# jseppanen/azalea

Measured on AMD Instinct MI355X. Metric: mcts_sims_per_sec, higher is better.
Workload: dtype f16x3 (fp32 operands split hi+lo f16, fp32 accumulate)

## Files before the change

azalea_amd/_lib.py:

```python
import ctypes as C
import logging
import os
import subprocess

_HERE = os.path.dirname(os.path.abspath(__file__))
LIB_PATH = os.path.join(_HERE, "libazx_hip.so")

MAX_BOARD = 13
CELL_STRIDE = 192
MAX_BATCH = 16
ROW_METRICS = 8


def record_bytes(cells):
    return (16 + 5 * cells + 15) // 16 * 16

EVAL_RESNET, EVAL_UNIFORM, EVAL_UNIFORM_HASH, EVAL_EXTERNAL = 0, 1, 2, 3
FLAG_NO_COMPACT = 1
FLAG_RANDOM_REFLECT = 2
FLAG_TOWER_F16 = 4
EEXTERNAL = -7


class AzxError(RuntimeError):
# ... 63 lines not shown
    "azx_get_status": (C.c_int, [_vp, _i32p]),
    "azx_get_tree_nodes": (C.c_int, [_vp, _i32p]),
    "azx_get_games": (C.c_int, [_vp, _i32p, _i32p, _i32p, _i32p]),
    "azx_advance": (C.c_int, [_vp, _i32p]),
    "azx_tree_dump": (C.c_int, [_vp, C.c_int, C.c_int, _i32p, _i32p, _i32p, _f32p, _f32p, _f32p, _i32p, _i32p]),
    "azx_forward": (C.c_int, [_vp, C.c_int, C.c_int, _i32p, _i32p, _f32p, _f32p]),
    "azx_hex_replay": (C.c_int, [C.c_int, C.c_int, C.c_int, _i32p, _i32p, C.c_int, _i32p, _i32p, _u64p, _i32p]),
    "azx_play": (C.c_int, [_vp, C.c_int64, C.c_int64, C.c_int64, _i32p, _i32p, _i32p, _f32p, _f32p, _i64p, C.POINTER(PlayStats)]),
    "azx_play_row_metrics": (C.c_int, [_vp, C.c_int64, _f32p, _i64p]),
    "azx_play_steps": (C.c_int, [_vp, C.c_int64, C.POINTER(PlayStats)]),
    "azx_replay_create": (C.c_int, [_vp, C.c_int64]),
    "azx_replay_state": (C.c_int, [_vp, _i64p, _i64p, _i64p]),
    "azx_replay_set_state": (C.c_int, [_vp, C.c_int64, C.c_int64]),
    "azx_replay_put": (C.c_int, [_vp, C.c_int64, _i32p, _i32p, _i32p, _f32p, _f32p]),
    "azx_replay_fill": (C.c_int, [_vp, C.c_int64, C.c_int64, _i64p, C.POINTER(PlayStats)]),
    "azx_play_device": (C.c_int, [_vp, C.c_int64, C.c_int64, _i64p, C.POINTER(PlayStats)]),
    "azx_rows_pack": (C.c_int, [_vp, C.c_int64, C.c_int64, _vp]),
    "azx_replay_put_records": (C.c_int, [_vp, C.c_int64, _vp]),
    "azx_replay_put_records_async": (C.c_int, [_vp, C.c_int64, _vp, _vp]),
    "azx_reserve_cus": (C.c_int, [_vp, C.c_int, C.POINTER(C.c_int)]),
    "azx_replay_collate": (C.c_int, [_vp, C.c_int64, _i64p, _vp, _vp, _vp, _vp, _vp, _vp, _i32p]),
    "azx_replay_collate_async": (C.c_int, [_vp, C.c_int64, _i64p, _vp, _vp, _vp, _vp, _vp, _vp, _vp]),
    "azx_replay_set_mover_view": (C.c_int, [_vp, C.c_int]),
    "azx_replay_set_reflect": (C.c_int, [_vp, C.c_int, C.c_uint64]),
    "azx_selftest_arith": (C.c_int, [C.c_int, C.c_int, _f32p, _f32p, _f32p, _f32p, _f32p]),
    "azx_selftest_divide": (C.c_int, [C.c_int, C.c_int, _f32p, _f32p, _f32p, _f32p]),
    "azx_selftest_dirichlet": (C.c_int, [C.c_int, C.c_double, C.c_int, C.c_int, C.c_uint32, _f32p]),
    "azx_debug_choose": (C.c_int, [_vp, _i32p, _f32p]),
    "azx_debug_counters": (C.c_int, [_vp, _u64p]),
    "azx_debug_counters_raw": (C.c_int, [_vp, _u64p, C.c_int64]),
    "azx_kernel_info": (C.c_int, [_vp, C.c_char_p, C.c_int]),
    "azx_debug_set_queue_cap": (C.c_int, [_vp, C.c_int64]),
    "azx_debug_stagger": (C.c_int, [_vp, _i32p]),
    "azx_stream": (_vp, [_vp]),
    "azx_set_external_evaluator": (C.c_int, [_vp, _vp, _vp]),
    "azx_match_create": (C.c_int, [_vp, _vp, C.POINTER(_vp)]),
    "azx_match_destroy": (None, [_vp]),
    "azx_match_play": (C.c_int, [_vp, C.c_int64, C.c_int64, C.POINTER(C.c_int8), C.POINTER(C.c_int16),
                                 C.POINTER(C.c_int16), C.POINTER(MatchStats)]),
    "azx_tournament_create": (C.c_int, [C.POINTER(_vp), C.c_int, C.POINTER(_vp)]),
    "azx_tournament_destroy": (None, [_vp]),
    "azx_tournament_play": (C.c_int, [_vp, C.c_int, _i32p, _i32p, C.c_int64, C.c_int64, C.c_int32,
                                      C.POINTER(C.c_int8), C.POINTER(C.c_int16), C.POINTER(C.c_int16),
                                      C.POINTER(MatchStats)]),
    "azx_match_set_harvest": (C.c_int, [_vp, C.c_int]),
    "azx_match_set_first_mover": (C.c_int, [_vp, C.c_int]),
    "azx_match_rows": (C.c_int, [_vp, _i64p]),
    "azx_tournament_set_harvest": (C.c_int, [_vp, C.c_int]),
    "azx_tournament_set_first_mover": (C.c_int, [_vp, C.c_int]),
    "azx_tournament_rows": (C.c_int, [_vp, _i64p]),
    "azx_rows_read": (C.c_int, [_vp, C.c_int64, C.c_int64, _i32p, _i32p, _i32p, _f32p, _f32p, _i64p]),
    "azx_openings_check": (C.c_int, [C.c_int, C.c_int, C.c_int, C.POINTER(C.c_int16), _i32p, _i32p, _i32p]),
    "azx_match_set_openings": (C.c_int, [_vp, C.c_int, C.c_int, C.POINTER(C.c_int16), _i32p]),
    "azx_tournament_set_openings": (C.c_int, [_vp, C.c_int, C.c_int, C.POINTER(C.c_int16), _i32p]),
    "azx_set_playout_cap": (C.c_int, [_vp, C.c_double, C.c_int]),
    "azx_playout_cap_is_full": (C.c_int, [C.c_uint64, C.c_int64, C.c_int, C.c_double]),
    "azx_playout_cap_stats": (C.c_int, [_vp, _i64p]),
    "azx_set_resign": (C.c_int, [_vp, C.c_double, C.c_int, C.c_double]),
    "azx_clear_resign": (C.c_int, [_vp]),
    "azx_resign_is_exempt": (C.c_int, [C.c_uint64, C.c_int64, C.c_double]),
    "azx_resign_stats": (C.c_int, [_vp, _i64p]),
    "azx_resign_value": (C.c_int, [_vp, C.POINTER(C.c_float)]),
    "azx_set_early_stop": (C.c_int, [_vp, C.c_int]),
    "azx_early_stop_stats": (C.c_int, [_vp, _i64p]),
    "azx_set_train_targets": (C.c_int, [_vp, C.c_int, C.c_float]),
    "azx_get_train_targets": (C.c_int, [_vp, C.POINTER(C.c_int), C.POINTER(C.c_float)]),
# ... 62 lines not shown
```

azalea_amd/csrc/azx_capi.cpp:

```cpp
#include <hip/hip_runtime.h>

#include <algorithm>
#include <cmath>
#include <cstdarg>
#include <cstdio>
#include <cstdlib>
#include <cstring>
#include <map>
#include <mutex>
#include <string>
#include <vector>

#include "../../include/azx.h"
#include "azx_dev.h"
#include "mcts_kernels.h"
#include "net.h"
#include "train.h"
#include "replay_kernels.h"
#include "ext_kernels.h"
#include "match_kernels.h"
#include "playout_cap.h"
#include "resign.h"

#ifndef AZX_SRC_SHA
#define AZX_SRC_SHA "unknown"
#endif

static thread_local std::string g_err;

static int fail(int code, const char *fmt, ...) {
    char buf[1024];
    va_list ap;
    va_start(ap, fmt);
    vsnprintf(buf, sizeof buf, fmt, ap);
    va_end(ap);
    g_err = buf;
    return code;
}

#define HIPCHECK(expr)                                                                    \
    do {                                                                                  \
        hipError_t _e = (expr);                                                           \
        if (_e != hipSuccess)                                                             \
            return fail(AZX_EHIP, "%s failed: %s (%s:%d)", #expr, hipGetErrorString(_e),  \
                        __FILE__, __LINE__);                                              \
    } while (0)

struct azx_engine {
    azx_config cfg;
    DevEngine d;
    hipStream_t stream = nullptr;
    int reserved_cus = 0;
    std::mutex alloc_mu;
    int num_batches = 0;
    int selects_per_search = 0;
// ... 400 lines not shown
    } else {
        snprintf(tree, sizeof tree, "k_mcts<%d,generic> (BEGIN / APPLY|SELECT / APPLY phases)", S);
        snprintf(play, sizeof play, "%s", !use_pipeline(e) ? "phases + k_choose + k_advance per move, one stream"
                                          : e->stagger     ? "phases + k_choose + k_advance per move, two half-pools on two streams half an evaluation apart (any tower)"
                                                           : "phases + k_choose + k_advance per move, two half-pools on two streams");
    }
    std::string text = std::string("tree=") + tree + "; play=" + play + "; net=" +
                       (e->net ? azx_net_kernel_info(e->net) : "none") +
                       "; switches: AZX_MCTS_GENERIC=" + (e->force_generic ? "1" : "0") +
                       " AZX_NO_PERSISTENT=" + (e->no_persistent ? "1" : "0") +
                       " AZX_PIPELINE=" + (e->pipeline ? "1" : "0") +
                       " AZX_PIPELINE_STAGGER=" + (e->stagger ? "1" : "0") +
                       " reserved_cus=" + std::to_string(e->reserved_cus) +
                       " reflect=" + ((d.flags & AZX_FLAG_RANDOM_REFLECT) ? "on" : "off") +
                       " cap=" + cap_text(e) +
                       " resign=" + resign_text(e) +
                       " estop=" + (e->estop_on ? "on" : "off") +
                       " targets=" + targets_text(e) +
                       "; src=" AZX_SRC_SHA;
    snprintf(buf, (size_t)cap, "%s", text.c_str());
    return (int)text.size();
}

extern "C" int azx_debug_stagger(azx_engine *e, int32_t *out4) {
    if (!e || !out4) return fail(AZX_EINVAL, "null argument");
    ENGINE_GUARD(e);
    memset(out4, 0, 4 * sizeof(int32_t));
    if (!e->stagger_ctr) return AZX_OK;
    HIPCHECK(hipMemcpyAsync(out4, e->stagger_ctr, 4 * sizeof(int32_t), hipMemcpyDeviceToHost, e->stream));
    HIPCHECK(hipStreamSynchronize(e->stream));
    return AZX_OK;
}

extern "C" int azx_debug_set_queue_cap(azx_engine *e, int64_t rows) {
    if (!e || rows < 0) return fail(AZX_EINVAL, "bad argument");
    e->dbg_qcap = rows;
    return AZX_OK;
}

static int check_net_range(azx_engine *e) {
    if (!e->net) return AZX_OK;
    int rc = azx_net_check_range(e->net, e->stream);
    if (rc) g_err = azx_net_error();
    return rc;
}

extern "C" int azx_debug_weights(azx_engine *e, int which, void *out, int64_t cap, int64_t *nbytes, char *name, int name_cap) {
    if (!e) return fail(AZX_EINVAL, "null engine");
    ENGINE_GUARD(e);
    if (!e->net) return fail(AZX_ESTATE, "engine was not created with AZX_EVAL_RESNET");
    int rc = azx_net_debug_weights(e->net, which, out, cap, nbytes, name, name_cap);
    if (rc) g_err = azx_net_error();
    return rc;
}

extern "C" int azx_set_weights(azx_engine *e, int n_tensors, const char *const *names,
                               const void *const *ptrs, const int64_t *counts, int on_device) {
    if (!e) return fail(AZX_EINVAL, "null engine");
    ENGINE_GUARD(e);
    if (!e->net) return fail(AZX_ESTATE, "engine was not created with AZX_EVAL_RESNET");
    int rc = azx_net_set_weights(e->net, n_tensors, names, ptrs, counts, on_device);
    if (rc) g_err = azx_net_error();
    return rc;
}

extern "C" int azx_set_prior_table(azx_engine *e, const float *prior_by_k, int count) {
// ... 2266 lines not shown
```

azalea_amd/csrc/net_kernels.hip:

```cpp
#include "net_priv.h"

#ifndef AZX_NET_ABLATE
#define AZX_NET_ABLATE 0
#endif
#ifndef AZX_SAT_TRACK
#define AZX_SAT_TRACK 1
#endif

#include <cmath>
#include <cstdio>
#include <cstdlib>
#include <cstring>
#include <map>
#include <string>
#include <type_traits>
#include <utility>
#include <vector>

typedef float f32x16 __attribute__((ext_vector_type(16)));

static thread_local std::string g_net_err;
const char *azx_net_error() { return g_net_err.c_str(); }

int azx_net_fail(int code, const char *msg) {
    g_net_err = msg;
    return code;
}
static int nfail(int code, const char *msg) { return azx_net_fail(code, msg); }


template <int C, int MT, int BPB, int MS, int NS>
__global__ __launch_bounds__(256) void k_tower_mfma(NetDev P, const uint8_t *__restrict__ ev_board,
                                                     const int32_t *__restrict__ n_eval_ptr,
// ... 165 lines not shown
#endif

#ifndef F16X3_BPB
#define F16X3_BPB 2
#endif
#ifndef AZX_S16_FENCE
#define AZX_S16_FENCE 1
#endif
typedef float f32x4 __attribute__((ext_vector_type(4)));

__global__ __launch_bounds__(F16X3_BPB * 128, 2) void k_tower_f16x3_s16(NetDev P, const uint8_t *__restrict__ ev_board,
                                                                        const int32_t *__restrict__ n_eval_ptr,
                                                                        int n_eval_host, float *__restrict__ act_out,
                                                                        float *__restrict__ hfeat) {
    constexpr int C = 64, ROWB = 272, MT = 4, NT = 4;
    extern __shared__ __align__(16) unsigned char smem[];
    const int n_eval = n_eval_ptr ? *n_eval_ptr : n_eval_host;
    const int e0 = blockIdx.x * F16X3_BPB;
    if (e0 >= n_eval) return;
    const int tid = threadIdx.x, lane = tid & 63, wave = __builtin_amdgcn_readfirstlane(tid >> 6);
    NT_DECL
    const int wb = wave >> 1, wh = wave & 1;
    const int N = P.N, ncells = P.ncells;
    const int e = e0 + wb;
    const bool live = e < n_eval;
    const int board_b = 128 * ROWB;
    const int zero_off = 0;
    const int x_off = 2 * ROWB + wb * board_b;
    unsigned char *X = smem + x_off;
    const int li = lane & 15, lh = lane >> 4;
    const int lrow = li < 8 ? li ^ 4 : li;
    const int lchunk = 128 * (lh & 1) + 16 * (lh >> 1);

    unsigned long long tapok = 0ull;
    int rbase[MT], ry_[MT], rx_[MT];
#pragma unroll
    for (int m = 0; m < MT; ++m) {
        const int r = 64 * wh + 16 * m + lrow;
        const int ry = r / N, rx = r - ry * N;
        ry_[m] = ry;
        rx_[m] = rx;
        rbase[m] = x_off + r * ROWB + lchunk;
#pragma unroll
        for (int tap = 0; tap < 9; ++tap) {
            const int yy = ry + tap / 3 - 1, xx = rx + tap % 3 - 1;
            if (r < ncells && yy >= 0 && yy < N && xx >= 0 && xx < N) tapok |= 1ull << (tap * 4 + m);
        }
    }
    uint32_t tapok_lo = (uint32_t)tapok, tapok_hi = (uint32_t)(tapok >> 32);
    auto act_offset = [&](int tap, int m) -> int {
        const int delta = ((tap / 3 - 1) * N + (tap % 3 - 1)) * ROWB;
        const uint32_t word = tap < 8 ? tapok_lo : tapok_hi;
        const int mask = (int)(word << (31 - ((tap * 4 + m) & 31))) >> 31;
        return (mask | 0xF0) & (rbase[m] + delta);
    };

    f32x4 res[MT][NT];
    auto load_bias = [&](const float *bias, float4 (&b4)[NT]) {
#pragma unroll
        for (int n = 0; n < NT; ++n) b4[n] = *reinterpret_cast<const float4 *>(bias + 16 * n + 4 * lh);
    };
    float satmax = 0.f;
    auto epilogue = [&](f32x4 (&acc)[MT][NT], const float4 (&bias4)[NT], auto kind_tag) {
        constexpr int kind = decltype(kind_tag)::value;
#pragma unroll
        for (int n = 0; n < NT; ++n) {
            const float4 b4 = bias4[n];
            const float bv[4] = {b4.x, b4.y, b4.z, b4.w};
#pragma unroll
            for (int m = 0; m < MT; ++m) {
                float v4[4];
#pragma unroll
                for (int j = 0; j < 4; ++j) {
                    float v = acc[m][n][j] + bv[j];
                    if (kind == 1) v += res[m][n][j];
                    v = fmaxf(v, 0.0f);
                    if (kind != 0) res[m][n][j] = v;
                    v4[j] = v;
                }
                if (AZX_SAT_TRACK) satmax = fmaxf(fmaxf(satmax, v4[0]), fmaxf(v4[1], fmaxf(v4[2], v4[3])));
                uint2 h4, l4;
                split2_f16(v4[0], v4[1], h4.x, l4.x);
                split2_f16(v4[2], v4[3], h4.y, l4.y);
                unsigned char *pw = X + (64 * wh + 16 * m + lrow) * ROWB + 128 * (lh >> 1) + 16 * n + 8 * (lh & 1);
                *reinterpret_cast<uint2 *>(pw) = h4;
                *reinterpret_cast<uint2 *>(pw + 64) = l4;
            }
        }
    };

    {
        const int NH = N + 2;
        unsigned char *cells = X + 121 * ROWB;
        const uint8_t *bd = ev_board + (size_t)(live ? e : n_eval - 1) * AZX_CELL_STRIDE;
        if (wh == 0) {
            for (int i = lane; i < NH * NH; i += 64) {
                const int y = i / NH - 1, x = i - (y + 1) * NH - 1;
                cells[i] = (y >= 0 && y < N && x >= 0 && x < N) ? bd[y * N + x] : (uint8_t)3;
            }
        }
        for (int i = tid; i < 2 * ROWB / 4; i += F16X3_BPB * 128) reinterpret_cast<uint32_t *>(smem + zero_off)[i] = 0u;
        __syncthreads();
        f32x4 acc[MT][NT];
#pragma unroll
        for (int m = 0; m < MT; ++m)
#pragma unroll
            for (int n = 0; n < NT; ++n) acc[m][n] = f32x4{0.f, 0.f, 0.f, 0.f};
        const uint4 *ws = reinterpret_cast<const uint4 *>(P.Ws16);
        f16x8 wfh[NT], wfl[NT];
#pragma unroll
        for (int n = 0; n < NT; ++n) {
            const uint4 qh = ws[(n * 2) * 64 + lane], ql = ws[(n * 2 + 1) * 64 + lane];
            wfh[n] = *reinterpret_cast<const f16x8 *>(&qh);
            wfl[n] = *reinterpret_cast<const f16x8 *>(&ql);
        }
#pragma unroll
        for (int m = 0; m < MT; ++m) {
            uint32_t onehot = 0u;
            if (64 * wh + 16 * m + lrow < ncells) {
                const unsigned char *c0 = cells + ry_[m] * NH + rx_[m];
#pragma unroll
                for (int tap = 0; tap < 9; ++tap) {
                    const uint32_t v = c0[(tap / 3) * NH + tap % 3];
                    onehot |= (v < 3u ? 1u : 0u) << (3 * tap + v);
                }
            }
            const uint32_t byte = (onehot >> (8 * lh)) & 0xffu;
            uint4 q;
            q.x = ((byte >> 0) & 1u) * 0x3C00u | ((byte >> 1) & 1u) * 0x3C000000u;
            q.y = ((byte >> 2) & 1u) * 0x3C00u | ((byte >> 3) & 1u) * 0x3C000000u;
            q.z = ((byte >> 4) & 1u) * 0x3C00u | ((byte >> 5) & 1u) * 0x3C000000u;
            q.w = ((byte >> 6) & 1u) * 0x3C00u | ((byte >> 7) & 1u) * 0x3C000000u;
            const f16x8 xf = *reinterpret_cast<const f16x8 *>(&q);
#pragma unroll
            for (int n = 0; n < NT; ++n) {
                acc[m][n] = __builtin_amdgcn_mfma_f32_16x16x32_f16(wfh[n], xf, acc[m][n], 0, 0, 0);
                acc[m][n] = __builtin_amdgcn_mfma_f32_16x16x32_f16(wfl[n], xf, acc[m][n], 0, 0, 0);
            }
        }
        float4 sb4[NT];
        load_bias(P.stem_b, sb4);
        __syncthreads();
        epilogue(acc, sb4, std::integral_constant<int, 2>{});
    }
    __syncthreads();
    NT_MARK(0)

    const uint4 *wsrc = reinterpret_cast<const uint4 *>(P.Wh16);
    int stage = 0;
    const int last_stage = P.layers * 18 - 1;
    f16x8 wh_[NT], wl_[NT];
    auto load_w = [&](int st, int nn, int part) {
        const uint4 qq = wsrc[(size_t)min(st, last_stage) * 512 + (nn * 2 + part) * 64 + lane];
        if (part) wl_[nn] = *reinterpret_cast<const f16x8 *>(&qq);
        else wh_[nn] = *reinterpret_cast<const f16x8 *>(&qq);
    };
#pragma unroll
    for (int i = 0; i < 4; ++i) load_w(0, i >> 1, i & 1);
    auto conv_layer = [&](int layer, auto residual_tag) {
        constexpr bool residual = decltype(residual_tag)::value;
        asm volatile("" : "+v"(tapok_lo), "+v"(tapok_hi), "+v"(rbase[0]), "+v"(rbase[1]), "+v"(rbase[2]), "+v"(rbase[3]));
        f32x4 acc[MT][NT];
#pragma unroll
        for (int m = 0; m < MT; ++m)
#pragma unroll
            for (int n = 0; n < NT; ++n) acc[m][n] = f32x4{0.f, 0.f, 0.f, 0.f};
        f16x8 xh[MT], xl[MT];
        auto load_x = [&](int tt, int mm, int part) {
            const unsigned char *pa = smem + act_offset(tt >> 1, mm) + (tt & 1) * 32 + part * 64;
            if (part) xl[mm] = *reinterpret_cast<const f16x8 *>(pa);
            else xh[mm] = *reinterpret_cast<const f16x8 *>(pa);
        };
#pragma unroll
        for (int m = 0; m < MT - 1; ++m) { load_x(0, m, 0); load_x(0, m, 1); }
#pragma unroll
        for (int t = 0; t < 18; ++t) {
#pragma unroll
            for (int h = 0; h < 2; ++h) {
#pragma unroll
                for (int q = 0; q < 24; ++q) {
                    const int m = q / 6, n = 2 * h + (q % 6) / 3, p = q % 3;
                    if (q == 1 || q == 4 || q == 7 || q == 10) {
                        const int idx = (q - 1) / 3;
                        if (h == 0) load_w(stage + t, 2 + (idx >> 1), idx & 1);
                        else load_w(stage + t + 1, idx >> 1, idx & 1);
                    } else if (h == 0 && (q == 13 || q == 16)) {
                        load_x(t, MT - 1, q == 16);
                    } else if (h == 1 && q >= 8 && (q % 6 == 2 || q % 6 == 5)) {
                        if (t + 1 < 18) load_x(t + 1, q / 6 - 1, q % 6 == 5);
                    }
                    const f16x8 wv = p == 1 ? wl_[n] : wh_[n];
                    const f16x8 xv = p == 2 ? xl[m] : xh[m];
                    acc[m][n] = __builtin_amdgcn_mfma_f32_16x16x32_f16(wv, xv, acc[m][n], 0, 0, 0);
#if AZX_S16_FENCE == 2
                    __builtin_amdgcn_sched_barrier(0);
#elif AZX_S16_FENCE == 1
                    if (q % 3 == 2) __builtin_amdgcn_sched_barrier(0);
#elif AZX_S16_FENCE == 3
                    if (q % 6 == 5) __builtin_amdgcn_sched_barrier(0);
#elif AZX_S16_FENCE == 4
                    if (q % 2 == 1) __builtin_amdgcn_sched_barrier(0);
#endif
                }
            }
        }
        stage += 18;
        float4 lb4[NT];
        load_bias(P.bias + layer * C, lb4);
        NT_MARK(2)
        __syncthreads();
        NT_MARK(3)
        epilogue(acc, lb4, std::integral_constant<int, residual ? 1 : 0>{});
        NT_MARK(4)
        __syncthreads();
        NT_MARK(5)
    };
    for (int blk = 0; blk < P.blocks; ++blk) {
        conv_layer(2 * blk, std::false_type{});
        conv_layer(2 * blk + 1, std::true_type{});
    }

    if (hfeat != nullptr) {
        const uint4 *whd = reinterpret_cast<const uint4 *>(P.Whd16);
        f16x8 ah[2], al[2];
#pragma unroll
        for (int ks = 0; ks < 2; ++ks) {
            const uint4 qh = whd[(ks * 2) * 64 + lane], ql = whd[(ks * 2 + 1) * 64 + lane];
            ah[ks] = *reinterpret_cast<const f16x8 *>(&qh);
            al[ks] = *reinterpret_cast<const f16x8 *>(&ql);
        }
        const float4 hb = *reinterpret_cast<const float4 *>(P.hbias16 + 4 * lh);
        const float hbv[4] = {hb.x, hb.y, hb.z, hb.w};
#pragma unroll
        for (int m = 0; m < MT; ++m) {
            f32x4 hacc = f32x4{0.f, 0.f, 0.f, 0.f};
#pragma unroll
            for (int ks = 0; ks < 2; ++ks) {
                const unsigned char *pa = smem + rbase[m] + ks * 32;
                const f16x8 xh = *reinterpret_cast<const f16x8 *>(pa), xl = *reinterpret_cast<const f16x8 *>(pa + 64);
                hacc = __builtin_amdgcn_mfma_f32_16x16x32_f16(ah[ks], xh, hacc, 0, 0, 0);
                hacc = __builtin_amdgcn_mfma_f32_16x16x32_f16(al[ks], xh, hacc, 0, 0, 0);
                hacc = __builtin_amdgcn_mfma_f32_16x16x32_f16(ah[ks], xl, hacc, 0, 0, 0);
            }
            const int row = 64 * wh + 16 * m + lrow;
            if (live && row < ncells) {
#pragma unroll
                for (int r = 0; r < 4; ++r) {
                    const int o = 4 * lh + r;
                    if (o < 6) hfeat[((size_t)e * 6 + o) * ncells + row] = fmaxf(hacc[r] + hbv[r], 0.0f);
                }
            }
        }
    }
    if (live && act_out != nullptr) {
        float *out = act_out + (size_t)e * ncells * C;
#pragma unroll
        for (int m = 0; m < MT; ++m) {
            const int row = 64 * wh + 16 * m + lrow;
            if (row < ncells) {
#pragma unroll
                for (int n = 0; n < NT; ++n)
                    *reinterpret_cast<float4 *>(out + row * C + 16 * n + 4 * lh) =
                        make_float4(res[m][n][0], res[m][n][1], res[m][n][2], res[m][n][3]);
            }
        }
    }
    if (satmax > 65504.0f) atomicOr(P.sat_flag, 1u);
    NT_MARK(6)
    NT_FLUSH
}

__global__ __launch_bounds__(F16X3_BPB * 128, 2) void k_tower_f16_s16(NetDev P, const uint8_t *__restrict__ ev_board,
                                                                      const int32_t *__restrict__ n_eval_ptr,
                                                                      int n_eval_host, float *__restrict__ hfeat) {
    constexpr int C = 64, ROWB = 272, MT = 4, NT = 4;
    extern __shared__ __align__(16) unsigned char smem[];
    const int n_eval = n_eval_ptr ? *n_eval_ptr : n_eval_host;
    const int e0 = blockIdx.x * F16X3_BPB;
    if (e0 >= n_eval) return;
    const int tid = threadIdx.x, lane = tid & 63, wave = __builtin_amdgcn_readfirstlane(tid >> 6);
    const int wb = wave >> 1, wh = wave & 1;
    const int N = P.N, ncells = P.ncells;
    const int e = e0 + wb;
    const bool live = e < n_eval;
    const int board_b = 128 * ROWB;
    const int zero_off = 0;
    const int x_off = 2 * ROWB + wb * board_b;
    unsigned char *X = smem + x_off;
    const int li = lane & 15, lh = lane >> 4;
    const int lrow = li < 8 ? li ^ 4 : li;
    const int lchunk = 128 * (lh & 1) + 16 * (lh >> 1);

// ... 1263 lines not shown
    AzxNet *net = new AzxNet();
    memset(&net->d, 0, sizeof net->d);
    net->d.N = N;
    net->d.ncells = N * N;
    net->d.C = chans;
    net->d.blocks = blocks;
    net->d.layers = 2 * blocks;
    net->max_evals = max_evals;
    net->stream = st;
    const int ncells = N * N;
    const char *force = getenv("AZX_TOWER");
    const bool want_fp32 = force && !strcmp(force, "fp32");
    const bool fused = azx_net_has_fused_tower(N, blocks, chans);
    const bool has_f16 = azx_net_has_f16_tower(N, blocks, chans);
    if (tower_f16 && (!has_f16 || want_fp32)) {
        delete net;
        return nfail(AZX_EINVAL, want_fp32 ? "net: the plain-f16 tower was asked for (AZX_FLAG_TOWER_F16) but AZX_TOWER=fp32 forces the fp32 tower"
                                           : "net: the plain-f16 tower (AZX_FLAG_TOWER_F16) exists for the fused tower's shapes (64 channels, at most "
                                             "121 cells) and the wide tower's (a multiple of 128 channels) only, with at least one block");
    }
    const bool want_f16 = tower_f16 || (force && !strcmp(force, "f16"));
    if (fused && !want_fp32) { net->tower_variant = 4; net->tower_f16 = want_f16; }
    else if (chans == 64 && ncells <= 128) net->tower_variant = 1;
    else if (chans == 64 && ncells <= 192) net->tower_variant = 2;
    else if (chans == 32 && ncells <= 192) net->tower_variant = 3;
    else if (has_wide_tower(N, chans) && !want_fp32) {
        net->tower_variant = 5;
        net->tower_f16 = want_f16 && blocks >= 1;
    }
    net->use_mfma = net->tower_variant != 0;
    { const char *v = getenv("AZX_WIDE_STREAMS"); net->opt_wsplit = std::min(4, std::max(1, v ? atoi(v) : 2)); }
    { const char *v = getenv("AZX_HEADS"); net->opt_heads_mfma = !(v && !strcmp(v, "valu")); }
    { const char *v = getenv("AZX_PACK"); net->pack_on_host = v && !strcmp(v, "host"); }
    {
        char b[260];
        const char *tower = "k_stem_generic + k_conv_generic (VALU)";
        if (net->tower_variant == 4) tower = net->tower_f16 ? "k_tower_f16_s16" : "k_tower_f16x3_s16";
        else if (net->tower_variant == 5) tower = net->tower_f16 ? "k_stem_wide_f16 + k_conv_wide_f16_s16 per layer"
                                                                 : "k_stem_wide_f16x3 + k_conv_wide_f16x3_s16 per layer";
        else if (net->tower_variant == 1) tower = "k_tower_mfma<64,4,2,1,2> (fp32 MFMA)";
        else if (net->tower_variant == 2) tower = "k_tower_mfma<64,6,1,2,2> (fp32 MFMA)";
        else if (net->tower_variant == 3) tower = "k_tower_mfma<32,6,2,2,1> (fp32 MFMA)";
        const bool hm = net->tower_variant == 4 && net->opt_heads_mfma && ncells <= 128;
        snprintf(b, sizeof b, "%s + %s (%dx%d on %dx%d; AZX_TOWER=%s AZX_WIDE_STREAMS=%d AZX_HEADS=%s AZX_PACK=%s)",
                 tower, hm ? "k_heads_mfma" : "k_heads", blocks, chans, N, N, want_fp32 ? "fp32" : net->tower_f16 ? "f16" : "default",
                 net->opt_wsplit, net->opt_heads_mfma ? "mfma" : "valu", net->pack_on_host ? "host" : "device");
        net->info = b;
    }
    const size_t E = max_evals;
    net->act = nalloc<float>(net, E * ncells * chans);
    net->logit = nalloc<float>(net, E * AZX_CELL_STRIDE);
    if (net->tower_variant == 4) net->hfeat = nalloc<float>(net, E * 6 * ncells);
    net->hb_board = nalloc<uint8_t>(net, E * AZX_CELL_STRIDE);
    net->hb_flip = nalloc<int32_t>(net, E);
    net->hb_value = nalloc<float>(net, E);
    if (!net->use_mfma) {
        net->act2 = nalloc<float>(net, E * ncells * chans);
        net->act3 = nalloc<float>(net, E * ncells * chans);
    }
    if (net->tower_variant == 5) {
        net->wideX = nalloc<unsigned short>(net, E * ncells * chans * 2);
        net->wideY = nalloc<unsigned short>(net, E * ncells * chans * 2);
    }
    if (!net->act || !net->logit || !net->hb_board || !net->hb_flip || !net->hb_value ||
        (!net->use_mfma && (!net->act2 || !net->act3)) || (net->tower_variant == 5 && (!net->wideX || !net->wideY))) {
        azx_net_destroy(net);
        return nfail(AZX_ENOMEM, "net: hipMalloc failed");
    }
    const int bpb = net->tower_variant == 2 ? 1 : 2;
    net->lds_bytes = (size_t)bpb * 2 * (ncells + 1) * (chans + 4) * sizeof(float);
    if (net->tower_variant == 4) net->lds_bytes = (size_t)F16X3_BPB * 128 * 272 + 2 * 272;
    if (net->tower_variant == 5) net->lds_bytes = (size_t)(ncells + 2) * WIDE_ROWB;
    net->d.sat_flag = nalloc<uint32_t>(net, 4);
    if (!net->d.sat_flag || hipDeviceSynchronize() != hipSuccess) {
        azx_net_destroy(net);
        return nfail(AZX_ENOMEM, "net: hipMalloc failed");
    }
    *out = net;
    return AZX_OK;
}

void azx_net_set_stream(AzxNet *net, hipStream_t st, const uint32_t *mask, int words) {
    if (!net) return;
    for (int i = 0; i < 3; ++i) {
        if (net->stream2[i]) { (void)hipStreamSynchronize(net->stream2[i]); (void)hipStreamDestroy(net->stream2[i]); }
        if (net->ev_join[i]) (void)hipEventDestroy(net->ev_join[i]);
        net->stream2[i] = nullptr;
        net->ev_join[i] = nullptr;
    }
    if (net->ev_fork) (void)hipEventDestroy(net->ev_fork);
    net->ev_fork = nullptr;
    net->streams_ok = false;
    net->cu_mask.assign(mask, mask + (mask ? words : 0));
    net->stream = st;
}

void azx_net_destroy(AzxNet *net) {
    if (net) {
        for (int i = 0; i < 3; ++i) {
            if (net->stream2[i]) { (void)hipStreamSynchronize(net->stream2[i]); (void)hipStreamDestroy(net->stream2[i]); }
            if (net->ev_join[i]) (void)hipEventDestroy(net->ev_join[i]);
            net->stream2[i] = nullptr;
            net->ev_join[i] = nullptr;
        }
        if (net->ev_fork) (void)hipEventDestroy(net->ev_fork);
        net->ev_fork = nullptr;
// ... 254 lines not shown
```

azalea_amd/csrc/net_priv.h:

```cpp
#pragma once
#include <hip/hip_runtime.h>
#include <stdint.h>

#include <algorithm>
#include <string>
#include <vector>

#include "net.h"

struct NetDev {
    int N, ncells, C, blocks, layers;
    const float *stemT;
    const float *stem_b;
    const unsigned short *Ws;
    const unsigned short *Ws16, *Wh16;
    const unsigned short *Whd16;
    const float *hbias16;
    const float *Wp;
    const float *Wg;
    const float *bias;
    const float *wv, *bv;
    const float *wp, *bp;
    const float *fc2T, *fc2b;
    const float *fc3w, *fc3b;
    const float *mfcT, *mfcb;
    const float *hmP, *hmV;
    int hm_lda;
    uint32_t *sat_flag;
};

#ifndef AZX_LO_BITS
#define AZX_LO_BITS 10
#endif
#define LO_MASK ((0xFFFFu << (10 - AZX_LO_BITS)) & 0xFFFFu)
#define LO_RND (AZX_LO_BITS < 10 ? (1u << (9 - AZX_LO_BITS)) : 0u)
static inline unsigned short lo_round_bits(unsigned short bits) {
    return (unsigned short)((bits + LO_RND) & LO_MASK);
}

struct AzxNet {
    NetDev d;
    int max_evals = 0;
    bool ready = false;
    bool use_mfma = false;
    hipStream_t stream = nullptr;
    std::vector<void *> allocs;
    float *act = nullptr, *act2 = nullptr, *act3 = nullptr;
    unsigned short *wideX = nullptr, *wideY = nullptr;
    float *logit = nullptr;
    float *hfeat = nullptr;
    uint8_t *hb_board = nullptr;
    int32_t *hb_flip = nullptr;
    float *hb_value = nullptr;
    size_t lds_bytes = 0;
    int tower_variant = 0;
    bool tower_f16 = false;
    hipStream_t stream2[3] = {nullptr, nullptr, nullptr};
    std::vector<uint32_t> cu_mask;
    hipEvent_t ev_fork = nullptr, ev_join[3] = {nullptr, nullptr, nullptr};
    bool streams_ok = false;
    int opt_wsplit = 2;
// ... 27 lines not shown
```

include/azx.h:

```cpp
#ifndef AZX_H
#define AZX_H

#include <stdint.h>

#ifdef __cplusplus
extern "C" {
#endif

#define AZX_MAX_BOARD 13
#define AZX_MAX_CELLS (AZX_MAX_BOARD * AZX_MAX_BOARD)
#define AZX_CELL_STRIDE 192
#define AZX_MAX_BATCH 16
#define AZX_ROW_METRICS 8
#define AZX_RECORD_BYTES(cells) ((size_t)((16 + 5 * (cells) + 15) / 16 * 16))

enum {
    AZX_OK = 0,
    AZX_EINVAL = -1,
    AZX_EHIP = -2,
    AZX_ENOMEM = -3,
    AZX_ESTATE = -4,
    AZX_ENODEV = -5,
    AZX_ERANGE = -6,
    AZX_EEXTERNAL = -7
// ... 152 lines not shown
int azx_playout_cap_stats(azx_engine *e, int64_t out4[4]);

int azx_set_resign(azx_engine *e, double threshold, int min_ply, double keep_prob);
int azx_clear_resign(azx_engine *e);
int azx_resign_is_exempt(uint64_t seed, int64_t uid, double keep_prob);
int azx_resign_stats(azx_engine *e, int64_t out8[8]);
int azx_resign_value(azx_engine *e, float *v);

int azx_set_early_stop(azx_engine *e, int on);
int azx_early_stop_stats(azx_engine *e, int64_t out4[4]);

#define AZX_ROWS_REFERENCE 0
#define AZX_ROWS_VISITS    1
int azx_set_train_targets(azx_engine *e, int policy_rows, float value_mix);
int azx_get_train_targets(azx_engine *e, int *policy_rows, float *value_mix);
int azx_train_targets_stats(azx_engine *e, int64_t out4[4]);

int azx_selftest_arith(int device, int n, const float *a, const float *b, float *sq, float *dv,
                       float *mul);

int azx_selftest_divide(int device, int n, const float *num, const float *den, float *quot,
                        float *sqrt_tab);

int azx_selftest_dirichlet(int device, double alpha, int k, int n_rows, uint32_t seed, float *out);

int azx_debug_choose(azx_engine *e, int32_t *move_id, float *moves_prob);

int azx_debug_counters(azx_engine *e, uint64_t *out16);
int azx_debug_counters_raw(azx_engine *e, uint64_t *out, int64_t n_games);

int azx_kernel_info(azx_engine *e, char *buf, int cap);
int azx_debug_set_queue_cap(azx_engine *e, int64_t rows);
int azx_debug_stagger(azx_engine *e, int32_t *out4);

typedef struct {
    int64_t games;
    int64_t wins[2];
    int64_t first_player_wins;
    int64_t voided;
    int64_t plies;
    double  seconds;
} azx_match_stats;
typedef struct azx_match azx_match;
int azx_match_create(azx_engine *a, azx_engine *b, azx_match **out);
void azx_match_destroy(azx_match *m);
int azx_match_play(azx_match *m, int64_t first_game, int64_t n_games, int8_t *outcome, int16_t *length,
                   int16_t *moves, azx_match_stats *stats);

int azx_match_set_harvest(azx_match *m, int on);
int azx_match_set_first_mover(azx_match *m, int mode);
int azx_match_rows(azx_match *m, int64_t *rows_out);

typedef struct azx_tournament azx_tournament;
int azx_tournament_create(azx_engine *const *engines, int n_engines, azx_tournament **out);
void azx_tournament_destroy(azx_tournament *t);
int azx_tournament_play(azx_tournament *t, int n_pairs, const int32_t *pair_a, const int32_t *pair_b,
                        int64_t first_game, int64_t rounds, int32_t tables_per_pair,
                        int8_t *outcome, int16_t *length, int16_t *moves, azx_match_stats *stats);
int azx_tournament_set_harvest(azx_tournament *t, int sink_engine);
int azx_tournament_set_first_mover(azx_tournament *t, int mode);
int azx_tournament_rows(azx_tournament *t, int64_t *rows_out);

int azx_openings_check(int board_size, int n_openings, int stride, const int16_t *moves, const int32_t *lengths,
                       int32_t *bad_opening, int32_t *bad_ply);
int azx_match_set_openings(azx_match *m, int n_openings, int stride, const int16_t *moves, const int32_t *lengths);
int azx_tournament_set_openings(azx_tournament *t, int n_openings, int stride, const int16_t *moves,
// ... 24 lines not shown
```

Measured before the change: 5.196 million.

## Remap tower rows so edge cells share a tile and skip padding taps

Builds a row permutation that puts 16 edge cells of one side (top, bottom, left, right) into the last M-tile of each wave, so that for some 3x3 taps every row in that tile reads padding. A per-wave skip mask tells the f16x3 tower kernel to drop those taps' MFMAs for the light tile. The kernel then reads row indices through a device tile map for the im2col gather, LDS writeback, heads output and activation output. This adds indirection loads and a branch inside the k-loop, and it lets rows from the two boards in a block mix within one wave.

```diff
diff --git a/azalea_amd/_lib.py b/azalea_amd/_lib.py
--- a/azalea_amd/_lib.py
+++ b/azalea_amd/_lib.py
@@ -119,6 +119,7 @@
     "azx_kernel_info": (C.c_int, [_vp, C.c_char_p, C.c_int]),
     "azx_debug_set_queue_cap": (C.c_int, [_vp, C.c_int64]),
     "azx_debug_stagger": (C.c_int, [_vp, _i32p]),
+    "azx_debug_tower_tiles": (C.c_int, [C.c_int, C.c_char_p, C.POINTER(C.c_uint8), C.POINTER(C.c_uint32), _i32p]),
     "azx_stream": (_vp, [_vp]),
     "azx_set_external_evaluator": (C.c_int, [_vp, _vp, _vp]),
     "azx_match_create": (C.c_int, [_vp, _vp, C.POINTER(_vp)]),
diff --git a/azalea_amd/csrc/azx_capi.cpp b/azalea_amd/csrc/azx_capi.cpp
--- a/azalea_amd/csrc/azx_capi.cpp
+++ b/azalea_amd/csrc/azx_capi.cpp
@@ -21,6 +21,7 @@
 #include "match_kernels.h"
 #include "playout_cap.h"
 #include "resign.h"
+#include "tower_tiles.h"
 
 #ifndef AZX_SRC_SHA
 #define AZX_SRC_SHA "unknown"
@@ -487,6 +488,19 @@
     return AZX_OK;
 }
 
+extern "C" int azx_debug_tower_tiles(int board_size, const char *map, uint8_t *rows256, uint32_t *skip4, int32_t *light_slot) {
+    if (!map || !rows256 || !skip4 || !light_slot) return fail(AZX_EINVAL, "null argument");
+    if (board_size < 2 || board_size * board_size > 121)
+        return fail(AZX_EINVAL, "tower tiles: board size %d outside the fused tower's 2..11", board_size);
+    if (strcmp(map, "edge") && strcmp(map, "rows")) return fail(AZX_EINVAL, "tower tiles: map '%s' is neither edge nor rows", map);
+    AzxTowerTiles t;
+    azx_tower_tiles_build(board_size, !strcmp(map, "edge"), &t);
+    memcpy(rows256, t.row, sizeof t.row);
+    for (int w = 0; w < 4; ++w) skip4[w] = t.skip[w];
+    *light_slot = AZX_TOWER_LIGHT_SLOT;
+    return t.edge;
+}
+
 extern "C" int azx_debug_set_queue_cap(azx_engine *e, int64_t rows) {
     if (!e || rows < 0) return fail(AZX_EINVAL, "bad argument");
     e->dbg_qcap = rows;
diff --git a/azalea_amd/csrc/net_kernels.hip b/azalea_amd/csrc/net_kernels.hip
--- a/azalea_amd/csrc/net_kernels.hip
+++ b/azalea_amd/csrc/net_kernels.hip
@@ -1,4 +1,5 @@
 #include "net_priv.h"
+#include "tower_tiles.h"
 
 #ifndef AZX_NET_ABLATE
 #define AZX_NET_ABLATE 0
@@ -230,15 +231,19 @@
     const int lrow = li < 8 ? li ^ 4 : li;
     const int lchunk = 128 * (lh & 1) + 16 * (lh >> 1);
 
+    constexpr int LT = AZX_TOWER_LIGHT_SLOT;
+    static_assert(LT == MT - 1, "the k-loop skips the lagging last tile");
+    const uint8_t *tmap = P.tile_map + 64 * wave + lrow;
+    const uint32_t skip = __builtin_amdgcn_readfirstlane((uint32_t)(P.tile_skip >> (9 * wave)) & 0x1ffu);
     unsigned long long tapok = 0ull;
-    int rbase[MT], ry_[MT], rx_[MT];
+    int rbase[MT], cell0_[MT];
 #pragma unroll
     for (int m = 0; m < MT; ++m) {
-        const int r = 64 * wh + 16 * m + lrow;
+        const int L = tmap[16 * m];
+        const int r = L & 127;
         const int ry = r / N, rx = r - ry * N;
-        ry_[m] = ry;
-        rx_[m] = rx;
-        rbase[m] = x_off + r * ROWB + lchunk;
+        cell0_[m] = r < ncells ? 2 * ROWB + (L >> 7) * board_b + 121 * ROWB + ry * (N + 2) + rx : -1;
+        rbase[m] = 2 * ROWB + L * ROWB + lchunk;
 #pragma unroll
         for (int tap = 0; tap < 9; ++tap) {
             const int yy = ry + tap / 3 - 1, xx = rx + tap % 3 - 1;
@@ -276,11 +281,14 @@
                     if (kind != 0) res[m][n][j] = v;
                     v4[j] = v;
                 }
-                if (AZX_SAT_TRACK) satmax = fmaxf(fmaxf(satmax, v4[0]), fmaxf(v4[1], fmaxf(v4[2], v4[3])));
+                if (AZX_SAT_TRACK) {
+                    satmax = fmaxf(fmaxf(satmax, v4[0]), fmaxf(v4[1], fmaxf(v4[2], v4[3])));
+                    asm volatile("" : "+v"(satmax));
+                }
                 uint2 h4, l4;
                 split2_f16(v4[0], v4[1], h4.x, l4.x);
                 split2_f16(v4[2], v4[3], h4.y, l4.y);
-                unsigned char *pw = X + (64 * wh + 16 * m + lrow) * ROWB + 128 * (lh >> 1) + 16 * n + 8 * (lh & 1);
+                unsigned char *pw = smem + rbase[m] + (112 * (lh >> 1) - 120 * (lh & 1)) + 16 * n;
                 *reinterpret_cast<uint2 *>(pw) = h4;
                 *reinterpret_cast<uint2 *>(pw + 64) = l4;
             }
@@ -315,8 +323,8 @@
 #pragma unroll
         for (int m = 0; m < MT; ++m) {
             uint32_t onehot = 0u;
-            if (64 * wh + 16 * m + lrow < ncells) {
-                const unsigned char *c0 = cells + ry_[m] * NH + rx_[m];
+            if (cell0_[m] >= 0) {
+                const unsigned char *c0 = smem + cell0_[m];
 #pragma unroll
                 for (int tap = 0; tap < 9; ++tap) {
                     const uint32_t v = c0[(tap / 3) * NH + tap % 3];
@@ -369,15 +377,35 @@
             if (part) xl[mm] = *reinterpret_cast<const f16x8 *>(pa);
             else xh[mm] = *reinterpret_cast<const f16x8 *>(pa);
         };
+        auto tap_skipped = [&](int tap) __attribute__((always_inline)) -> bool {
+            uint32_t s = skip;
+            asm volatile("" : "+s"(s));
+            return (s >> tap) & 1u;
+        };
+        auto fence = [&](int q) __attribute__((always_inline)) {
+#if AZX_S16_FENCE == 2
+            __builtin_amdgcn_sched_barrier(0);
+#elif AZX_S16_FENCE == 1
+            if (q % 3 == 2) __builtin_amdgcn_sched_barrier(0);
+#elif AZX_S16_FENCE == 3
+            if (q % 6 == 5) __builtin_amdgcn_sched_barrier(0);
+#elif AZX_S16_FENCE == 4
+            if (q % 2 == 1) __builtin_amdgcn_sched_barrier(0);
+#endif
+        };
+        auto mfma1 = [&](int h, int m, int j) __attribute__((always_inline)) {
+            const int n = 2 * h + j / 3, p = j % 3;
+            const f16x8 wv = p == 1 ? wl_[n] : wh_[n];
+            const f16x8 xv = p == 2 ? xl[m] : xh[m];
+            acc[m][n] = __builtin_amdgcn_mfma_f32_16x16x32_f16(wv, xv, acc[m][n], 0, 0, 0);
+        };
 #pragma unroll
         for (int m = 0; m < MT - 1; ++m) { load_x(0, m, 0); load_x(0, m, 1); }
 #pragma unroll
         for (int t = 0; t < 18; ++t) {
 #pragma unroll
             for (int h = 0; h < 2; ++h) {
-#pragma unroll
-                for (int q = 0; q < 24; ++q) {
-                    const int m = q / 6, n = 2 * h + (q % 6) / 3, p = q % 3;
+                auto step_q = [&](int q) __attribute__((always_inline)) {
                     if (q == 1 || q == 4 || q == 7 || q == 10) {
                         const int idx = (q - 1) / 3;
                         if (h == 0) load_w(stage + t, 2 + (idx >> 1), idx & 1);
@@ -387,18 +415,17 @@
                     } else if (h == 1 && q >= 8 && (q % 6 == 2 || q % 6 == 5)) {
                         if (t + 1 < 18) load_x(t + 1, q / 6 - 1, q % 6 == 5);
                     }
-                    const f16x8 wv = p == 1 ? wl_[n] : wh_[n];
-                    const f16x8 xv = p == 2 ? xl[m] : xh[m];
-                    acc[m][n] = __builtin_amdgcn_mfma_f32_16x16x32_f16(wv, xv, acc[m][n], 0, 0, 0);
-#if AZX_S16_FENCE == 2
-                    __builtin_amdgcn_sched_barrier(0);
-#elif AZX_S16_FENCE == 1
-                    if (q % 3 == 2) __builtin_amdgcn_sched_barrier(0);
-#elif AZX_S16_FENCE == 3
-                    if (q % 6 == 5) __builtin_amdgcn_sched_barrier(0);
-#elif AZX_S16_FENCE == 4
-                    if (q % 2 == 1) __builtin_amdgcn_sched_barrier(0);
-#endif
+                    mfma1(h, q / 6, q % 6);
+                    fence(q);
+                };
+#pragma unroll
+                for (int q = 0; q < 6 * LT; ++q) step_q(q);
+                if (!tap_skipped(t >> 1)) {
+#pragma unroll
+                    for (int q = 6 * LT; q < 24; ++q) step_q(q);
+                } else if (h == 1 && t + 1 < 18) {
+                    load_x(t + 1, MT - 2, 0);
+                    load_x(t + 1, MT - 2, 1);
                 }
             }
         }
@@ -440,22 +467,22 @@
                 hacc = __builtin_amdgcn_mfma_f32_16x16x32_f16(al[ks], xh, hacc, 0, 0, 0);
                 hacc = __builtin_amdgcn_mfma_f32_16x16x32_f16(ah[ks], xl, hacc, 0, 0, 0);
             }
-            const int row = 64 * wh + 16 * m + lrow;
-            if (live && row < ncells) {
+            const int L = tmap[16 * m], row = L & 127, el = e0 + (L >> 7);
+            if (el < n_eval && row < ncells) {
 #pragma unroll
                 for (int r = 0; r < 4; ++r) {
                     const int o = 4 * lh + r;
-                    if (o < 6) hfeat[((size_t)e * 6 + o) * ncells + row] = fmaxf(hacc[r] + hbv[r], 0.0f);
-                }
-            }
-        }
-    }
-    if (live && act_out != nullptr) {
-        float *out = act_out + (size_t)e * ncells * C;
+                    if (o < 6) hfeat[((size_t)el * 6 + o) * ncells + row] = fmaxf(hacc[r] + hbv[r], 0.0f);
+                }
+            }
+        }
+    }
+    if (act_out != nullptr) {
 #pragma unroll
         for (int m = 0; m < MT; ++m) {
-            const int row = 64 * wh + 16 * m + lrow;
-            if (row < ncells) {
+            const int L = tmap[16 * m], row = L & 127, el = e0 + (L >> 7);
+            float *out = act_out + (size_t)el * ncells * C;
+            if (el < n_eval && row < ncells) {
 #pragma unroll
                 for (int n = 0; n < NT; ++n)
                     *reinterpret_cast<float4 *>(out + row * C + 16 * n + 4 * lh) =
@@ -1785,8 +1812,13 @@
     { const char *v = getenv("AZX_WIDE_STREAMS"); net->opt_wsplit = std::min(4, std::max(1, v ? atoi(v) : 2)); }
     { const char *v = getenv("AZX_HEADS"); net->opt_heads_mfma = !(v && !strcmp(v, "valu")); }
     { const char *v = getenv("AZX_PACK"); net->pack_on_host = v && !strcmp(v, "host"); }
+    const bool x3 = net->tower_variant == 4 && !net->tower_f16;
+    AzxTowerTiles tiles;
+    bool want_edge = true;
+    { const char *v = getenv("AZX_TOWER_TILES"); want_edge = !(v && !strcmp(v, "rows")); }
+    azx_tower_tiles_build(N, x3 && want_edge, &tiles);
     {
-        char b[260];
+        char b[320];
         const char *tower = "k_stem_generic + k_conv_generic (VALU)";
         if (net->tower_variant == 4) tower = net->tower_f16 ? "k_tower_f16_s16" : "k_tower_f16x3_s16";
         else if (net->tower_variant == 5) tower = net->tower_f16 ? "k_stem_wide_f16 + k_conv_wide_f16_s16 per layer"
@@ -1795,8 +1827,9 @@
         else if (net->tower_variant == 2) tower = "k_tower_mfma<64,6,1,2,2> (fp32 MFMA)";
         else if (net->tower_variant == 3) tower = "k_tower_mfma<32,6,2,2,1> (fp32 MFMA)";
         const bool hm = net->tower_variant == 4 && net->opt_heads_mfma && ncells <= 128;
-        snprintf(b, sizeof b, "%s + %s (%dx%d on %dx%d; AZX_TOWER=%s AZX_WIDE_STREAMS=%d AZX_HEADS=%s AZX_PACK=%s)",
+        snprintf(b, sizeof b, "%s + %s (%dx%d on %dx%d; AZX_TOWER=%s AZX_TOWER_TILES=%s AZX_WIDE_STREAMS=%d AZX_HEADS=%s AZX_PACK=%s)",
                  tower, hm ? "k_heads_mfma" : "k_heads", blocks, chans, N, N, want_fp32 ? "fp32" : net->tower_f16 ? "f16" : "default",
+                 want_edge && (tiles.edge || !x3) ? "edge" : "rows",
                  net->opt_wsplit, net->opt_heads_mfma ? "mfma" : "valu", net->pack_on_host ? "host" : "device");
         net->info = b;
     }
@@ -1825,6 +1858,16 @@
     if (net->tower_variant == 4) net->lds_bytes = (size_t)F16X3_BPB * 128 * 272 + 2 * 272;
     if (net->tower_variant == 5) net->lds_bytes = (size_t)(ncells + 2) * WIDE_ROWB;
     net->d.sat_flag = nalloc<uint32_t>(net, 4);
+    if (x3) {
+        uint8_t *tm = nalloc<uint8_t>(net, sizeof tiles.row);
+        if (tm && hipMemcpy(tm, tiles.row, sizeof tiles.row, hipMemcpyHostToDevice) != hipSuccess) tm = nullptr;
+        if (!tm) {
+            azx_net_destroy(net);
+            return nfail(AZX_ENOMEM, "net: the tower's tile map could not be put on the device");
+        }
+        net->d.tile_map = tm;
+        for (int w = 0; w < 4; ++w) net->d.tile_skip |= (unsigned long long)(tiles.skip[w] & 0x1ffu) << (9 * w);
+    }
     if (!net->d.sat_flag || hipDeviceSynchronize() != hipSuccess) {
         azx_net_destroy(net);
         return nfail(AZX_ENOMEM, "net: hipMalloc failed");
diff --git a/azalea_amd/csrc/net_priv.h b/azalea_amd/csrc/net_priv.h
--- a/azalea_amd/csrc/net_priv.h
+++ b/azalea_amd/csrc/net_priv.h
@@ -27,6 +27,8 @@
     const float *hmP, *hmV;
     int hm_lda;
     uint32_t *sat_flag;
+    const uint8_t *tile_map;
+    unsigned long long tile_skip;
 };
 
 #ifndef AZX_LO_BITS
diff --git a/azalea_amd/csrc/tower_tiles.h b/azalea_amd/csrc/tower_tiles.h
--- /dev/null
+++ b/azalea_amd/csrc/tower_tiles.h
@@ -0,0 +1,91 @@
+#pragma once
+#include <stdint.h>
+
+#define AZX_TOWER_LIGHT_SLOT 3
+
+struct AzxTowerTiles {
+    uint8_t row[256];
+    uint32_t skip[4];
+    int edge;
+};
+
+static inline bool azx_tile_tap_is_padding(int N, int L, int tap) {
+    const int cell = L & 127;
+    if (cell >= N * N) return true;
+    const int y = cell / N + tap / 3 - 1, x = cell % N + tap % 3 - 1;
+    return y < 0 || y >= N || x < 0 || x >= N;
+}
+
+static inline void azx_tower_tiles_rows(AzxTowerTiles *t) {
+    for (int i = 0; i < 256; ++i) t->row[i] = (uint8_t)i;
+    for (int w = 0; w < 4; ++w) t->skip[w] = 0u;
+    t->edge = 0;
+}
+
+static inline void azx_tile_slot_keys(int L, int tile_row, int *k1, int *k2) {
+    const bool a = (tile_row & 4) == 0;
+    *k1 = (L + (a ? 8 : 0)) & 15;
+    *k2 = (L + (a ? 0 : 8)) & 15;
+}
+
+static inline void azx_tower_tiles_build(int N, int edge, AzxTowerTiles *t) {
+    azx_tower_tiles_rows(t);
+    if (!edge || N < 2 || N * N > 121) return;
+    const int ncells = N * N;
+    int cls[256];
+    for (int L = 0; L < 256; ++L) {
+        const int cell = L & 127, y = cell / N, x = cell % N;
+        cls[L] = cell >= ncells ? 5 : y == 0 ? 0 : y == N - 1 ? 1 : x == 0 ? 2 : x == N - 1 ? 3 : 4;
+    }
+    bool used[256] = {false};
+    int light[4][16];
+    for (int c = 0; c < 4; ++c) {
+        int nres[16] = {0}, chosen[16];
+        for (int k = 0; k < 16; ++k) {
+            int best = -1;
+            for (int pass = 0; pass < 2 && best < 0; ++pass)
+                for (int L = 0; L < 256; ++L)
+                    if (!used[L] && cls[L] == (pass ? 5 : c) && (best < 0 || nres[L & 15] < nres[best & 15])) best = L;
+            if (best < 0) { azx_tower_tiles_rows(t); return; }
+            used[best] = true;
+            ++nres[best & 15];
+            chosen[k] = best;
+        }
+        int n1[16] = {0}, n2[16] = {0};
+        bool taken[16] = {false};
+        for (int k = 0; k < 16; ++k) {
+            int best = -1, best_cost = 0;
+            for (int r = 0; r < 16; ++r) {
+                if (taken[r]) continue;
+                int k1, k2;
+                azx_tile_slot_keys(chosen[k], r, &k1, &k2);
+                const int cost = n1[k1] + n2[k2];
+                if (best < 0 || cost < best_cost) { best = r; best_cost = cost; }
+            }
+            int k1, k2;
+            azx_tile_slot_keys(chosen[k], best, &k1, &k2);
+            ++n1[k1];
+            ++n2[k2];
+            taken[best] = true;
+            light[c][best] = chosen[k];
+        }
+    }
+    int next = 0;
+    for (int w = 0; w < 4; ++w)
+        for (int m = 0; m < 4; ++m)
+            for (int r = 0; r < 16; ++r) {
+                if (m == AZX_TOWER_LIGHT_SLOT) { t->row[64 * w + 16 * m + r] = (uint8_t)light[w][r]; continue; }
+                while (used[next]) ++next;
+                t->row[64 * w + 16 * m + r] = (uint8_t)next++;
+            }
+    for (int w = 0; w < 4; ++w) {
+        uint32_t mask = 0u;
+        for (int tap = 0; tap < 9; ++tap) {
+            bool all = true;
+            for (int r = 0; r < 16; ++r) all = all && azx_tile_tap_is_padding(N, t->row[64 * w + 16 * AZX_TOWER_LIGHT_SLOT + r], tap);
+            if (all) mask |= 1u << tap;
+        }
+        t->skip[w] = mask;
+    }
+    t->edge = 1;
+}
diff --git a/include/azx.h b/include/azx.h
--- a/include/azx.h
+++ b/include/azx.h
@@ -208,6 +208,7 @@
 int azx_kernel_info(azx_engine *e, char *buf, int cap);
 int azx_debug_set_queue_cap(azx_engine *e, int64_t rows);
 int azx_debug_stagger(azx_engine *e, int32_t *out4);
+int azx_debug_tower_tiles(int board_size, const char *map, uint8_t *rows256, uint32_t *skip4, int32_t *light_slot);
 
 typedef struct {
     int64_t games;
```

After: 5.352 million (median of 6 runs). 1.03x the previous value.
